# lucidrains/progen

Hardware: NVIDIA H100
Metric: tokens_per_sec (higher is better)
Workload: dtype bf16

## Files before the change

include/progen_b200.h:

```cpp
#ifndef PROGEN_B200_H
#define PROGEN_B200_H
#include <stdint.h>

#ifdef __cplusplus
extern "C" {
#endif

#define PROGEN_F32 0
#define PROGEN_BF16 1

#define PROGEN_BACKEND_SIMT 0
#define PROGEN_BACKEND_TC 1

#define PROGEN_EPI_STORE 0
#define PROGEN_EPI_ROTARY 1
#define PROGEN_EPI_RESIDUAL 2
#define PROGEN_EPI_GLU 3
#define PROGEN_EPI_GELU 4
#define PROGEN_EPI_GLU_BWD 5
#define PROGEN_EPI_GELU_BWD 6
#define PROGEN_EPI_ACCUM 7

const char* progen_version(void);
const char* progen_last_error(void);
// ... 5 lines not shown
  int32_t a_mn_major, b_mn_major;
  int32_t batch;
  int32_t batch_reduce;
  int32_t causal;
  int32_t split_k;
  int32_t in_dtype, out_dtype, epi_kind, backend;
  int32_t seq_len, dim_head;
  int32_t atomic, tril, tril_rows;
  int64_t lda, ldb;
  int64_t a_batch_rows, b_batch_rows, d_batch_rows;
  int64_t ldo, ldo2, ldaux;
  const void* A;
  const void* B;
  void* out;
  void* out2;
  const float* bias;
  const void* aux;
  const float* rot_sin;
  const float* rot_cos;
  float* colsum;
  int64_t lda2, ldb2;
  const void* A2;
  const void* B2;
  int32_t K2, a2_mn_major, b2_mn_major, _pad_tail;
} progen_gemm_t;

int progen_gemm(const progen_gemm_t* desc, void* stream);

int progen_embed_fwd(const int* tokens, const float* table, float* x, long long T, int d, int V, void* stream);
int progen_embed_bwd(const int* tokens, const float* dx, float* dtable, long long T, int d, int V, void* stream);

int progen_ln_shift_fwd(const void* x, long long ldx, int x_dtype, const float* scale, void* y, long long ldy, int y_dtype,
                        float* mean, float* rstd, long long T, int d, int seq_len, int shift, void* stream);
int progen_ln_shift_bwd(const void* dy, long long lddy, int act_dtype, const void* x, long long ldx, int x_dtype,
                        const float* scale, const float* mean, const float* rstd, float* dres, void* dout, long long ldo,
                        float* dscale, float* dres_colsum, long long T, int d, int seq_len, int shift, int residual,
                        void* stream);

int progen_colsum(const void* in, long long ld, int dtype, float* out, long long T, int N, void* stream);

int progen_ce_fwd_bwd(const void* logits, int dtype, const int* labels, float* weights, float* loss, void* dlogits,
                      int dlogits_dtype, int B, int n, int V, float inv_batch, void* stream);

int progen_token_logprob(const void* logits, int dtype, const int* labels, float* logp, float* seq_ll, float* seq_count,
                         int B, int n, int V, void* stream);
int progen_preference_head(const void* logits, int dtype, const int* labels, const float* ref_ll, float* logp, float* seq_ll,
                           float* seq_count, float* weights, float* stats, float* loss, float* ce_scratch, void* dlogits,
// ... 143 lines not shown
```

progen_b200/csrc/api.cu:

```cuda
#include <stdarg.h>
#include "gemm.h"
#include "../../include/progen_b200.h"

static thread_local char g_err[1024] = "";
unsigned long long g_progen_launches = 0;

void progen_set_error(const char* fmt, ...) {
  va_list ap;
  va_start(ap, fmt);
  vsnprintf(g_err, sizeof(g_err), fmt, ap);
  va_end(ap);
}

extern "C" {

const char* progen_version(void) { return "progen_b200 0.1.0 (sm_90a; wgmma/TMA GEMM, CUDA " CUDA_VERSION_STR ")"; }

const char* progen_last_error(void) { return g_err; }

long long progen_launch_count(void) { return (long long)__atomic_load_n(&g_progen_launches, __ATOMIC_RELAXED); }

int progen_device_check(void) {
  int dev = 0;
  PG_CUDA(cudaGetDevice(&dev));
// ... 6 lines not shown
  }
  return PROGEN_OK;
}

int progen_gemm(const progen_gemm_t* d, void* stream) {
  PG_CHECK_ARG(d != nullptr);
  GemmArgs g;
  g.M = d->M; g.N = d->N; g.K = d->K;
  g.A = d->A; g.lda = d->lda; g.a_mn_major = d->a_mn_major;
  g.B = d->B; g.ldb = d->ldb; g.b_mn_major = d->b_mn_major;
  g.batch = d->batch < 1 ? 1 : d->batch;
  g.a_batch_rows = d->a_batch_rows; g.b_batch_rows = d->b_batch_rows; g.d_batch_rows = d->d_batch_rows;
  g.batch_reduce = d->batch_reduce; g.causal = d->causal; g.split_k = d->split_k < 1 ? 1 : d->split_k;
  g.in_dtype = d->in_dtype; g.out_dtype = d->out_dtype; g.epi_kind = d->epi_kind;
  g.epi.out = d->out; g.epi.ldo = d->ldo; g.epi.out2 = d->out2; g.epi.ldo2 = d->ldo2;
  g.epi.bias = d->bias; g.epi.aux = d->aux; g.epi.ldaux = d->ldaux;
  g.epi.rot_sin = d->rot_sin; g.epi.rot_cos = d->rot_cos;
  g.epi.seq_len = d->seq_len > 0 ? d->seq_len : 1; g.epi.dim_head = d->dim_head > 0 ? d->dim_head : 2;
  g.epi.atomic = d->atomic; g.epi.tril = d->tril; g.epi.tril_rows = d->tril_rows > 0 ? d->tril_rows : 1;
  g.epi.colsum = d->colsum;
  g.K2 = d->K2;
  g.A2 = d->A2; g.lda2 = d->lda2; g.a2_mn_major = d->a2_mn_major;
  g.B2 = d->B2; g.ldb2 = d->ldb2; g.b2_mn_major = d->b2_mn_major;
  PG_CHECK_ARG(g.epi_kind >= 0 && g.epi_kind < EPI_NUM_KINDS);
  PG_CHECK_ARG(g.epi.out != nullptr);
  PG_CHECK_ARG(!g.epi.colsum || g.epi_kind == EPI_GLU_BWD || g.epi_kind == EPI_GELU_BWD);
  if (g.epi_kind == EPI_GLU || g.epi_kind == EPI_GELU) PG_CHECK_ARG(g.epi.bias != nullptr);
  if (g.epi_kind == EPI_GLU_BWD || g.epi_kind == EPI_GELU_BWD) PG_CHECK_ARG(g.epi.aux != nullptr);
  if (g.epi_kind == EPI_ROTARY) PG_CHECK_ARG(g.epi.rot_sin && g.epi.rot_cos && d->seq_len > 0 && d->dim_head > 0 && d->dim_head % 2 == 0);
  if (d->backend == PROGEN_BACKEND_TC) return gemm_tc_launch(g, (cudaStream_t)stream);
  if (d->backend == PROGEN_BACKEND_SIMT) return gemm_simt_launch(g, (cudaStream_t)stream);
  progen_set_error("progen_gemm: unknown backend %d", d->backend);
  return PROGEN_ERR_ARG;
}

}
```

progen_b200/csrc/gemm.h:

```cpp
#pragma once
#include "epilogues.cuh"

struct GemmArgs {
  int M, N, K;
  const void* A; long long lda; int a_mn_major;
  const void* B; long long ldb; int b_mn_major;
  int batch; long long a_batch_rows; long long b_batch_rows; long long d_batch_rows;
  int batch_reduce;
  int causal;
  int split_k;
  int in_dtype;
  int out_dtype;
  int epi_kind;
  EpiArgs epi;
  const void* A2; long long lda2; int a2_mn_major;
  const void* B2; long long ldb2; int b2_mn_major;
  int K2;
};

#define PG_CHECK_TAIL(a)                                                                                               \
  do {                                                                                                                 \
    PG_CHECK_ARG((a).K2 >= 0);                                                                                         \
    if ((a).K2 > 0) {                                                                                                  \
      PG_CHECK_ARG((a).A2 != nullptr && (a).B2 != nullptr);                                                            \
      PG_CHECK_ARG((a).split_k == 1 && !(a).causal && (a).batch == 1 && !(a).batch_reduce && (a).epi_kind != EPI_ACCUM); \
    }                                                                                                                  \
  } while (0)

int gemm_tc_launch(const GemmArgs& g, cudaStream_t stream);
int gemm_simt_launch(const GemmArgs& g, cudaStream_t stream);
```

progen_b200/csrc/gemm_tc.cu:

```cuda
#include <cuda.h>
#include <algorithm>
#include <mutex>
#include <unordered_map>
#include "gemm.h"
#include "tc_ptx.cuh"

namespace {

using namespace tc;

constexpr int BM = 128;
constexpr int BN = 128;
constexpr int BK = 64;
constexpr int WG_K = 16;
constexpr int THREADS = 384;
constexpr int A_BYTES = BM * BK * 2;
constexpr int B_BYTES = BN * BK * 2;
constexpr int STAGE_BYTES = A_BYTES + B_BYTES;
constexpr int STAGES = 4;
constexpr int EPI_ROWS = 64;
constexpr int EPI_ITEMS = EPI_ROWS * (BN / 8) / 128;
constexpr int CS_LD = BN + 4;
constexpr int CS_BYTES = EPI_ROWS * CS_LD * 4;
constexpr int SMEM_TOTAL = 1024  + STAGES * STAGE_BYTES + 2 * CS_BYTES + 2 * STAGES * 8;
static_assert(SMEM_TOTAL <= 227 * 1024, "H100: 227 KiB of shared memory per block");
constexpr int BAR_TURN = 1, BAR_EPI = 3;
constexpr int PRODUCER_REGS = 40, CONSUMER_REGS = 232;
static_assert(128 * PRODUCER_REGS + 256 * CONSUMER_REGS <= 65536, "register file");

__device__ __forceinline__ void named_bar_sync(int id, int n) { asm volatile("bar.sync %0, %1;" ::"r"(id), "r"(n) : "memory"); }
__device__ __forceinline__ void named_bar_arrive(int id, int n) { asm volatile("bar.arrive %0, %1;" ::"r"(id), "r"(n) : "memory"); }
template <int R> __device__ __forceinline__ void setmaxnreg_dec() { asm volatile("setmaxnreg.dec.sync.aligned.u32 %0;" ::"n"(R)); }
template <int R> __device__ __forceinline__ void setmaxnreg_inc() { asm volatile("setmaxnreg.inc.sync.aligned.u32 %0;" ::"n"(R)); }

struct GemmDev {
  int M, N, K;
  int batch, batch_reduce;
  int a_batch_rows, b_batch_rows;
  long long d_batch_rows;
  int causal, split_k;
  EpiArgs epi;
  int K2;
};

struct TileInfo {
  int z, m0, n0, kb_begin, kb_end;
  int kb_main;
};

template <bool TAIL>
__device__ __forceinline__ void decode_tile(const GemmDev& g, int t, TileInfo& ti) {
  const int m_tiles = (g.M + BM - 1) / BM;
  const int n_tiles = (g.N + BN - 1) / BN;
  const int per_z = g.split_k * m_tiles * n_tiles;
  ti.z = t / per_z;
  int r = t - ti.z * per_z;
  const int ks = r / (m_tiles * n_tiles);
  r -= ks * (m_tiles * n_tiles);
  ti.m0 = (r / n_tiles) * BM;
  ti.n0 = (r % n_tiles) * BN;
  const int kb_total = (g.K + BK - 1) / BK;
  int b = 0, e = kb_total;
  if (g.causal == 1) e = min(kb_total, (ti.m0 + BM + BK - 1) / BK);
  if (g.causal == 2) b = min(kb_total, ti.m0 / BK);
  if (g.split_k > 1) {
    const int per = (kb_total + g.split_k - 1) / g.split_k;
    b = min(kb_total, ks * per);
    e = min(kb_total, b + per);
  }
  ti.kb_begin = b;
  ti.kb_end = e;
  if constexpr (TAIL) {
    ti.kb_main = e;
    ti.kb_end = e + (g.K2 + BK - 1) / BK;
  }
}

template <bool A_MN, bool B_MN, int KIND, typename TO, bool TAIL>
__global__ void __launch_bounds__(THREADS, 1)
gemm_tc_kernel(const __grid_constant__ CUtensorMap tma_a, const __grid_constant__ CUtensorMap tma_b,
               const __grid_constant__ CUtensorMap tma_a2, const __grid_constant__ CUtensorMap tma_b2, const GemmDev g,
               const int tiles) {
  extern __shared__ uint8_t smem_raw[];
  const uint32_t raw_u32 = smem_u32(smem_raw);
  const uint32_t smem_base = (raw_u32 + 1023u) & ~1023u;
  const uint32_t cs_base = smem_base + STAGES * STAGE_BYTES;
  const uint32_t bar_base = cs_base + 2 * CS_BYTES;
  auto full_bar = [&](int s) { return bar_base + 8u * s; };
  auto empty_bar = [&](int s) { return bar_base + 8u * (STAGES + s); };

  const int wg = threadIdx.x >> 7;
  if (threadIdx.x == 0) {
    prefetch_tensormap(&tma_a);
    prefetch_tensormap(&tma_b);
    if constexpr (TAIL) {
      prefetch_tensormap(&tma_a2);
      prefetch_tensormap(&tma_b2);
    }
    for (int s = 0; s < STAGES; ++s) {
      mbar_init(full_bar(s), 1);
      mbar_init(empty_bar(s), 1);
    }
    fence_barrier_init();
  }
  __syncthreads();

  int stage = 0;
  uint32_t phase = 0;
  auto advance = [&](int n) {
    stage += n;
    phase ^= (uint32_t)(stage / STAGES) & 1u;
    stage %= STAGES;
  };

  if (wg == 0) {
    setmaxnreg_dec<PRODUCER_REGS>();
    if (threadIdx.x == 0) {
      for (int t = blockIdx.x; t < tiles; t += gridDim.x) {
        TileInfo ti;
        decode_tile<TAIL>(g, t, ti);
        const int a_row0 = ti.z * g.a_batch_rows;
        const int b_row0 = ti.z * g.b_batch_rows;
        for (int kb = ti.kb_begin; kb < ti.kb_end; ++kb) {
          mbar_wait(empty_bar(stage), phase ^ 1);
          const uint32_t sa = smem_base + stage * STAGE_BYTES;
          const uint32_t sb = sa + A_BYTES;
          mbar_expect_tx(full_bar(stage), STAGE_BYTES);
          if (TAIL && kb >= ti.kb_main) {
            const int k0 = (kb - ti.kb_main) * BK;
            if constexpr (!A_MN) {
              tma_load_2d(sa, &tma_a2, full_bar(stage), k0, ti.m0);
            } else {
#pragma unroll
              for (int i = 0; i < BM / 64; ++i) tma_load_2d(sa + i * 8192, &tma_a2, full_bar(stage), ti.m0 + 64 * i, k0);
            }
            if constexpr (!B_MN) {
              tma_load_2d(sb, &tma_b2, full_bar(stage), k0, ti.n0);
            } else {
#pragma unroll
              for (int i = 0; i < BN / 64; ++i) tma_load_2d(sb + i * 8192, &tma_b2, full_bar(stage), ti.n0 + 64 * i, k0);
            }
            advance(1);
            continue;
          }
          const int k0 = kb * BK;
          if constexpr (!A_MN) {
            tma_load_2d(sa, &tma_a, full_bar(stage), k0, a_row0 + ti.m0);
          } else {
#pragma unroll
            for (int i = 0; i < BM / 64; ++i)
              tma_load_2d(sa + i * 8192, &tma_a, full_bar(stage), ti.m0 + 64 * i, a_row0 + k0);
          }
          if constexpr (!B_MN) {
            tma_load_2d(sb, &tma_b, full_bar(stage), k0, b_row0 + ti.n0);
          } else {
#pragma unroll
            for (int i = 0; i < BN / 64; ++i)
              tma_load_2d(sb + i * 8192, &tma_b, full_bar(stage), ti.n0 + 64 * i, b_row0 + k0);
          }
          advance(1);
        }
      }
    }
    return;
  }

  setmaxnreg_inc<CONSUMER_REGS>();
  const int c = wg - 1;
  const int tid = threadIdx.x & 127;
  float* cs = reinterpret_cast<float*>(smem_raw + (cs_base - raw_u32)) + c * (CS_BYTES / 4);
  for (int p = 0, t = blockIdx.x; t < tiles; ++p, t += gridDim.x) {
    TileInfo ti;
    decode_tile<TAIL>(g, t, ti);
    if ((p & 1) != c) {
      advance(ti.kb_end - ti.kb_begin);
      continue;
    }
    float acc[2][64];
#pragma unroll
    for (int i = 0; i < 64; ++i) acc[0][i] = acc[1][i] = 0.f;
    if (p > 0) named_bar_sync(BAR_TURN + c, 256);
    int prev = -1;
    for (int kb = ti.kb_begin; kb < ti.kb_end; ++kb) {
      mbar_wait(full_bar(stage), phase);
      const uint32_t sa = smem_base + stage * STAGE_BYTES;
      const uint64_t adesc0 = make_smem_desc<A_MN>(sa), adesc1 = make_smem_desc<A_MN>(sa + 8192);
      const uint64_t bdesc = make_smem_desc<B_MN>(sa + A_BYTES);
      constexpr uint32_t a_step = A_MN ? (2048 >> 4) : (32 >> 4), b_step = B_MN ? (2048 >> 4) : (32 >> 4);
      fence_regs(acc[0]);
      fence_regs(acc[1]);
      wgmma_fence();
#pragma unroll
      for (int k = 0; k < BK / WG_K; ++k) {
        wgmma_m64n128k16_bf16<A_MN ? 1 : 0, B_MN ? 1 : 0>(acc[0], adesc0 + (uint64_t)(k * a_step), bdesc + (uint64_t)(k * b_step));
        wgmma_m64n128k16_bf16<A_MN ? 1 : 0, B_MN ? 1 : 0>(acc[1], adesc1 + (uint64_t)(k * a_step), bdesc + (uint64_t)(k * b_step));
      }
      wgmma_commit();
      fence_regs(acc[0]);
      fence_regs(acc[1]);
      wgmma_wait<1>();
      if (prev >= 0 && tid == 0) mbar_arrive(empty_bar(prev));
      prev = stage;
      advance(1);
    }
    if (t + (int)gridDim.x < tiles) named_bar_arrive(BAR_TURN + (c ^ 1), 256);

    const int w = tid >> 5, lane = tid & 31;
    const int r0 = 16 * w + (lane >> 2), c0 = 2 * (lane & 3);
// ... 121 lines not shown
  cuuint64_t dims[2] = {inner, outer};
  cuuint64_t strides[1] = {row_stride_elems * elem_bytes};
  const CUtensorMapSwizzle sw = swizzle == 128 ? CU_TENSOR_MAP_SWIZZLE_128B : swizzle == 64 ? CU_TENSOR_MAP_SWIZZLE_64B
                              : swizzle == 32 ? CU_TENSOR_MAP_SWIZZLE_32B : CU_TENSOR_MAP_SWIZZLE_NONE;
  cuuint32_t box[2] = {box_inner, box_outer};
  cuuint32_t estr[2] = {1, 1};
  CUtensorMap m;
  CUresult r = fn(&m, elem_bytes == 4 ? CU_TENSOR_MAP_DATA_TYPE_FLOAT32 : CU_TENSOR_MAP_DATA_TYPE_BFLOAT16, 2,
                  const_cast<void*>(ptr), dims, strides, box, estr, CU_TENSOR_MAP_INTERLEAVE_NONE, sw, CU_TENSOR_MAP_L2_PROMOTION_L2_256B,
                  CU_TENSOR_MAP_FLOAT_OOB_FILL_NONE);
  if (r != CUDA_SUCCESS) {
    progen_set_error("cuTensorMapEncodeTiled failed (CUresult %d) ptr=%p inner=%llu outer=%llu stride=%llu box=%ux%u", (int)r,
                     ptr, (unsigned long long)inner, (unsigned long long)outer, (unsigned long long)row_stride_elems,
                     box_inner, box_outer);
    return PROGEN_ERR_CUDA;
  }
  if (cache.size() > 4096) cache.clear();
  cache.emplace(key, m);
  *out = m;
  return PROGEN_OK;
}


template <bool A_MN, bool B_MN, int KIND, typename TO, bool TAIL>
int launch_inst(const CUtensorMap& ta, const CUtensorMap& tb, const CUtensorMap& ta2, const CUtensorMap& tb2,
                const GemmDev& gd, int tiles, cudaStream_t stream) {
  auto kern = gemm_tc_kernel<A_MN, B_MN, KIND, TO, TAIL>;
  static bool attr_set = false;
  if (!attr_set) {
    PG_CUDA(cudaFuncSetAttribute(kern, cudaFuncAttributeMaxDynamicSharedMemorySize, SMEM_TOTAL));
    attr_set = true;
  }
  kern<<<std::min(tiles, pg_num_sms()), THREADS, SMEM_TOTAL, stream>>>(ta, tb, ta2, tb2, gd, tiles);
  PG_LAUNCH_CHECK();
  return PROGEN_OK;
}

}

int pg_tensor_map_2d_bf16(const void* ptr, uint64_t inner, uint64_t outer, uint64_t row_stride_elems, uint32_t box_inner,
                          uint32_t box_outer, CUtensorMap* out) {
  return get_tensor_map(ptr, inner, outer, row_stride_elems, box_inner, box_outer, out);
}

int gemm_tc_launch(const GemmArgs& a, cudaStream_t stream) {
  PG_CHECK_ARG(a.in_dtype == PG_BF16);
  PG_CHECK_ARG(a.M > 0 && a.N > 0 && a.K > 0 && a.batch >= 1 && a.split_k >= 1);
  PG_CHECK_ARG(a.N % 8 == 0);
  PG_CHECK_ARG(a.K % BK == 0);
  PG_CHECK_ARG(a.lda % 8 == 0 && a.ldb % 8 == 0);
  PG_CHECK_ARG((reinterpret_cast<uintptr_t>(a.A) & 15) == 0 && (reinterpret_cast<uintptr_t>(a.B) & 15) == 0);
  PG_CHECK_ARG(!(a.split_k > 1 && a.causal));
  if (a.epi_kind == EPI_ROTARY) PG_CHECK_ARG(a.epi.seq_len % 32 == 0);
  PG_CHECK_ARG((reinterpret_cast<uintptr_t>(a.epi.colsum) & 15) == 0);
  PG_CHECK_ARG(!(a.split_k > 1 || a.batch_reduce) || (a.epi_kind == EPI_ACCUM && a.epi.atomic));
  PG_CHECK_TAIL(a);
  const bool tail = a.K2 > 0;
  if (tail) {
    PG_CHECK_ARG(a.K2 % 8 == 0 && a.lda2 % 8 == 0 && a.ldb2 % 8 == 0);
    PG_CHECK_ARG(a.a2_mn_major == a.a_mn_major && a.b2_mn_major == a.b_mn_major);
    PG_CHECK_ARG((reinterpret_cast<uintptr_t>(a.A2) & 15) == 0 && (reinterpret_cast<uintptr_t>(a.B2) & 15) == 0);
  }

  const uint64_t a_rows = (a.batch > 1 && a.a_batch_rows > 0) ? (uint64_t)a.a_batch_rows * a.batch
                                                              : (uint64_t)(a.a_mn_major ? a.K : a.M);
  const uint64_t b_rows = (a.batch > 1 && a.b_batch_rows > 0) ? (uint64_t)a.b_batch_rows * a.batch
                                                              : (uint64_t)(a.b_mn_major ? a.K : a.N);
  CUtensorMap ta, tb;
  int rc;
  if (!a.a_mn_major) rc = get_tensor_map(a.A, a.K, a_rows, a.lda, BK, BM, &ta);
  else               rc = get_tensor_map(a.A, a.M, a_rows, a.lda, 64, BK, &ta);
  if (rc) return rc;
  if (!a.b_mn_major) rc = get_tensor_map(a.B, a.K, b_rows, a.ldb, BK, BN, &tb);
  else               rc = get_tensor_map(a.B, a.N, b_rows, a.ldb, 64, BK, &tb);
  if (rc) return rc;
  CUtensorMap ta2 = ta, tb2 = tb;
  if (tail) {
    if (!a.a_mn_major) rc = get_tensor_map(a.A2, a.K2, a.M, a.lda2, BK, BM, &ta2);
    else               rc = get_tensor_map(a.A2, a.M, a.K2, a.lda2, 64, BK, &ta2);
    if (rc) return rc;
    if (!a.b_mn_major) rc = get_tensor_map(a.B2, a.K2, a.N, a.ldb2, BK, BN, &tb2);
    else               rc = get_tensor_map(a.B2, a.N, a.K2, a.ldb2, 64, BK, &tb2);
    if (rc) return rc;
  }

  GemmDev gd;
  gd.M = a.M; gd.N = a.N; gd.K = a.K;
  gd.batch = a.batch; gd.batch_reduce = a.batch_reduce;
  gd.a_batch_rows = (int)a.a_batch_rows; gd.b_batch_rows = (int)a.b_batch_rows; gd.d_batch_rows = a.d_batch_rows;
  gd.causal = a.causal; gd.split_k = a.split_k;
  gd.epi = a.epi;
  gd.K2 = a.K2;
  const long long tiles = (long long)a.batch * a.split_k * ((a.M + BM - 1) / BM) * ((a.N + BN - 1) / BN);
  PG_CHECK_ARG(tiles < (1ll << 31));

  const int am = a.a_mn_major ? 1 : 0, bm = a.b_mn_major ? 1 : 0;
  const bool obf = a.out_dtype == PG_BF16;
#define TC_CASE(AM, BMJ, KIND, TO)                                                                       \
  return tail ? launch_inst<AM, BMJ, KIND, TO, true>(ta, tb, ta2, tb2, gd, (int)tiles, stream)            \
              : launch_inst<AM, BMJ, KIND, TO, false>(ta, tb, ta2, tb2, gd, (int)tiles, stream)
  switch (a.epi_kind) {
    case EPI_STORE:
      if (!am && bm) { if (obf) TC_CASE(false, true, EPI_STORE, bf16); else TC_CASE(false, true, EPI_STORE, float); }
      if (!am && !bm) { if (obf) TC_CASE(false, false, EPI_STORE, bf16); else TC_CASE(false, false, EPI_STORE, float); }
      if (am && bm) { if (obf) TC_CASE(true, true, EPI_STORE, bf16); else TC_CASE(true, true, EPI_STORE, float); }
      break;
    case EPI_ROTARY:
      if (!am && bm && obf) TC_CASE(false, true, EPI_ROTARY, bf16);
      break;
    case EPI_RESIDUAL:
      if (!am && bm) TC_CASE(false, true, EPI_RESIDUAL, float);
      break;
    case EPI_GLU:
      if (!am && bm && obf) TC_CASE(false, true, EPI_GLU, bf16);
      break;
    case EPI_GELU:
      if (!am && bm && obf) TC_CASE(false, true, EPI_GELU, bf16);
      break;
    case EPI_GLU_BWD:
      if (!am && !bm && obf) TC_CASE(false, false, EPI_GLU_BWD, bf16);
      break;
    case EPI_GELU_BWD:
      if (!am && !bm && obf) TC_CASE(false, false, EPI_GELU_BWD, bf16);
      break;
    case EPI_ACCUM:
      if (am && bm) return launch_inst<true, true, EPI_ACCUM, float, false>(ta, tb, ta2, tb2, gd, (int)tiles, stream);
      if (!am && !bm) return launch_inst<false, false, EPI_ACCUM, float, false>(ta, tb, ta2, tb2, gd, (int)tiles, stream);
      break;
    default: break;
  }
#undef TC_CASE
  progen_set_error("gemm_tc: unsupported combination epi=%d a_mn=%d b_mn=%d out=%d", a.epi_kind, am, bm, a.out_dtype);
  return PROGEN_ERR_UNSUPPORTED;
}
```

progen_b200/csrc/tc_ptx.cuh:

```cuda
#pragma once
#include <cuda.h>
#include "common.cuh"

namespace tc {

__device__ __forceinline__ uint32_t smem_u32(const void* p) { return (uint32_t)__cvta_generic_to_shared(p); }

__device__ __forceinline__ void mbar_init(uint32_t bar, uint32_t count) {
  asm volatile("mbarrier.init.shared::cta.b64 [%0], %1;" ::"r"(bar), "r"(count) : "memory");
}
__device__ __forceinline__ void mbar_expect_tx(uint32_t bar, uint32_t bytes) {
  asm volatile("mbarrier.arrive.expect_tx.shared::cta.b64 _, [%0], %1;" ::"r"(bar), "r"(bytes) : "memory");
}
__device__ __forceinline__ void mbar_arrive(uint32_t bar) {
  asm volatile("mbarrier.arrive.shared::cta.b64 _, [%0];" ::"r"(bar) : "memory");
}
__device__ __forceinline__ void mbar_wait(uint32_t bar, uint32_t parity) {
  uint32_t ok = 0, spins = 0;
  do {
    asm volatile(
        "{\n\t.reg .pred p;\n\t"
        "mbarrier.try_wait.parity.shared::cta.b64 p, [%1], %2;\n\t"
        "selp.u32 %0, 1, 0, p;\n\t}"
        : "=r"(ok) : "r"(bar), "r"(parity) : "memory");
// ... 30 lines not shown
  for (int i = 0; i < R; ++i) asm volatile("" : "+f"(d[i])::"memory");
}

template <int TA, int TB>
__device__ __forceinline__ void wgmma_m64n128k16_bf16(float (&d)[64], uint64_t adesc, uint64_t bdesc) {
  asm volatile(
      "{\n\t"
      "wgmma.mma_async.sync.aligned.m64n128k16.f32.bf16.bf16 "
      "{%0, %1, %2, %3, %4, %5, %6, %7, %8, %9, %10, %11, %12, %13, %14, %15, %16, %17, %18, %19, %20, %21, %22, %23, "
      "%24, %25, %26, %27, %28, %29, %30, %31, %32, %33, %34, %35, %36, %37, %38, %39, %40, %41, %42, %43, %44, %45, %46, "
      "%47, %48, %49, %50, %51, %52, %53, %54, %55, %56, %57, %58, %59, %60, %61, %62, %63}, "
      "%64, %65, 1, 1, 1, %66, %67;\n\t}"
      : "+f"(d[0]), "+f"(d[1]), "+f"(d[2]), "+f"(d[3]), "+f"(d[4]), "+f"(d[5]), "+f"(d[6]), "+f"(d[7]), "+f"(d[8]),
        "+f"(d[9]), "+f"(d[10]), "+f"(d[11]), "+f"(d[12]), "+f"(d[13]), "+f"(d[14]), "+f"(d[15]), "+f"(d[16]),
        "+f"(d[17]), "+f"(d[18]), "+f"(d[19]), "+f"(d[20]), "+f"(d[21]), "+f"(d[22]), "+f"(d[23]), "+f"(d[24]),
        "+f"(d[25]), "+f"(d[26]), "+f"(d[27]), "+f"(d[28]), "+f"(d[29]), "+f"(d[30]), "+f"(d[31]), "+f"(d[32]),
        "+f"(d[33]), "+f"(d[34]), "+f"(d[35]), "+f"(d[36]), "+f"(d[37]), "+f"(d[38]), "+f"(d[39]), "+f"(d[40]),
        "+f"(d[41]), "+f"(d[42]), "+f"(d[43]), "+f"(d[44]), "+f"(d[45]), "+f"(d[46]), "+f"(d[47]), "+f"(d[48]),
        "+f"(d[49]), "+f"(d[50]), "+f"(d[51]), "+f"(d[52]), "+f"(d[53]), "+f"(d[54]), "+f"(d[55]), "+f"(d[56]),
        "+f"(d[57]), "+f"(d[58]), "+f"(d[59]), "+f"(d[60]), "+f"(d[61]), "+f"(d[62]), "+f"(d[63])
      : "l"(adesc), "l"(bdesc), "n"(TA), "n"(TB));
}

template <int TB>
__device__ __forceinline__ void wgmma_m64n64k16_ss(float (&d)[32], uint64_t adesc, uint64_t bdesc) {
  asm volatile(
      "{\n\t"
      "wgmma.mma_async.sync.aligned.m64n64k16.f32.bf16.bf16 "
      "{%0, %1, %2, %3, %4, %5, %6, %7, %8, %9, %10, %11, %12, %13, %14, %15, %16, %17, %18, %19, %20, %21, %22, %23, %24, %25, %26, %27, %28, %29, %30, %31}, "
      "%32, %33, 1, 1, 1, 0, %34;\n\t}"
      : "+f"(d[0]), "+f"(d[1]), "+f"(d[2]), "+f"(d[3]), "+f"(d[4]), "+f"(d[5]), "+f"(d[6]), "+f"(d[7]), "+f"(d[8]), "+f"(d[9]), "+f"(d[10]), "+f"(d[11]), "+f"(d[12]), "+f"(d[13]), "+f"(d[14]), "+f"(d[15]), "+f"(d[16]), "+f"(d[17]), "+f"(d[18]), "+f"(d[19]), "+f"(d[20]), "+f"(d[21]), "+f"(d[22]), "+f"(d[23]), "+f"(d[24]), "+f"(d[25]), "+f"(d[26]), "+f"(d[27]), "+f"(d[28]), "+f"(d[29]), "+f"(d[30]), "+f"(d[31])
      : "l"(adesc), "l"(bdesc), "n"(TB));
}
template <int TB>
__device__ __forceinline__ void wgmma_m64n64k16_rs(float (&d)[32], const uint32_t (&a)[4], uint64_t bdesc) {
  asm volatile(
      "{\n\t"
      "wgmma.mma_async.sync.aligned.m64n64k16.f32.bf16.bf16 "
      "{%0, %1, %2, %3, %4, %5, %6, %7, %8, %9, %10, %11, %12, %13, %14, %15, %16, %17, %18, %19, %20, %21, %22, %23, %24, %25, %26, %27, %28, %29, %30, %31}, "
      "{%32, %33, %34, %35}, %36, 1, 1, 1, %37;\n\t}"
      : "+f"(d[0]), "+f"(d[1]), "+f"(d[2]), "+f"(d[3]), "+f"(d[4]), "+f"(d[5]), "+f"(d[6]), "+f"(d[7]), "+f"(d[8]), "+f"(d[9]), "+f"(d[10]), "+f"(d[11]), "+f"(d[12]), "+f"(d[13]), "+f"(d[14]), "+f"(d[15]), "+f"(d[16]), "+f"(d[17]), "+f"(d[18]), "+f"(d[19]), "+f"(d[20]), "+f"(d[21]), "+f"(d[22]), "+f"(d[23]), "+f"(d[24]), "+f"(d[25]), "+f"(d[26]), "+f"(d[27]), "+f"(d[28]), "+f"(d[29]), "+f"(d[30]), "+f"(d[31])
      : "r"(a[0]), "r"(a[1]), "r"(a[2]), "r"(a[3]), "l"(bdesc), "n"(TB));
}

}

// ... 3 lines not shown
```

progen_b200/engine.py:

```python
import math
import numpy as np
import torch

from . import lib as L

P = 'pro_gen_base/~/'
ALIGN = 64


CUT_ALIGN = 128


def counted_length(labels):
    labels = np.asarray(labels)
    n = labels.shape[1]
    pad = labels == 0
    first = np.where(pad.any(1), pad.argmax(1), n)
    last = np.where((~pad).any(1), n - 1 - (~pad)[:, ::-1].argmax(1), -1)
    return np.minimum(n, np.maximum(first, last) + 1)


def cut_length(labels):
    n = np.asarray(labels).shape[1]
    need = int(counted_length(labels).max()) if len(labels) else 1
    return min(n, -(-need // CUT_ALIGN) * CUT_ALIGN)


def check_length(labels, length, what):
    labels = np.asarray(labels)
    n = labels.shape[1]
    if length is None:
        return cut_length(labels)
    if isinstance(length, (bool, np.bool_)) or not isinstance(length, (int, np.integer)) or \
# ... 317 lines not shown
        if lo is None:
            return {}
        seg = lo.layout.seg
        g, A = lo.g[:acts.T], seg(lo.lp, module, 'lora_a')
        self.dgrad_gemm(dy, N, seg(lo.lp, module, 'lora_b'), lo.r, g, acts=acts)
        self.wgrad_gemm(lo.u[module][:acts.T], lo.r, dy, N, seg(lo.grads, module, 'lora_b'), acts=acts)
        self.wgrad_gemm(x, K, g, lo.r, seg(lo.grads, module, 'lora_a'), acts=acts)
        return dict(A2=g, lda2=lo.r, B2=A, ldb2=lo.r, K2=lo.r)

    def fwd_gemm(self, x, K, w, N, out, epi=L.EPI_STORE, out_dtype=None, acts=None, **kw):
        self._mm(M=(acts or self.acts).T, N=N, K=K, A=x, lda=K, B=w, ldb=N, b_mn=True, out=out, ldo=kw.pop('ldo', N), epi=epi,
                 out_dtype=self.act_dt if out_dtype is None else out_dtype, **kw)

    def dgrad_gemm(self, dy, N_out, w, K_in, out, epi=L.EPI_STORE, acts=None, **kw):
        self._mm(M=(acts or self.acts).T, N=K_in, K=N_out, A=dy, lda=N_out, B=w, ldb=N_out, out=out, ldo=kw.pop('ldo', K_in), epi=epi,
                 out_dtype=self.act_dt, **kw)

    def wgrad_gemm(self, x, K_in, dy, N_out, dw, acts=None):
        split = self.wgrad_split(K_in, N_out, acts) if self.backend == L.BACKEND_TC else 1
        self._mm(M=K_in, N=N_out, K=(acts or self.acts).T, A=x, lda=K_in, a_mn=True, B=dy, ldb=N_out, b_mn=True, out=dw, ldo=N_out,
                 epi=L.EPI_ACCUM, out_dtype=L.F32, split_k=split, atomic=split > 1)

    def wgrad_split(self, K_in, N_out, acts=None):
        tiles = ((K_in + 127) // 128) * ((N_out + 127) // 128)
        fill = lambda s: tiles * s / (-(-tiles * s // self.num_sms) * self.num_sms)
        return max(range(1, min(8, max(1, (acts or self.acts).T // 64)) + 1), key=lambda s: (round(fill(s), 6), -s))

    def colsum(self, t, N, out, ld=None, acts=None):
        L.check(self.lib.progen_colsum(t.data_ptr(), N if ld is None else ld, L.dt(t), out.data_ptr(), (acts or self.acts).T, N,
                                       L.stream()), 'colsum')

    def ln_fwd(self, x, ldx, scale, y, ldy, mean, rstd, dcols, shift, acts=None):
        a = acts or self.acts
        L.check(self.lib.progen_ln_shift_fwd(x.data_ptr(), ldx, L.dt(x), scale.data_ptr(), y.data_ptr(), ldy, L.dt(y),
                                             mean.data_ptr(), rstd.data_ptr(), a.T, dcols, a.n, int(shift), L.stream()),
                'ln_fwd')

    def forward(self, ids):
        B = ids.shape[0]
        self.ensure_batch(B)
        self.tok.copy_(torch.as_tensor(ids).reshape(-1).to(device=self.dev, dtype=torch.int32), non_blocking=True)
        self._forward_device()
        return self.logits

    def prefill(self, ids, P, sink):
        Bs = ids.shape[0]
        if tuple(ids.shape[1:]) != (self.n,) or not 0 < P < self.n:
            raise L.ProgenError(f'prefill: ids must be (B, {self.n}) and 0 < P < {self.n}')
        acts = self.inference_acts(Bs)
# ... 426 lines not shown
```

progen_b200/lib.py:

```python
import ctypes as C
import os
import torch

F32, BF16 = 0, 1
BACKEND_SIMT, BACKEND_TC = 0, 1
EPI_STORE, EPI_ROTARY, EPI_RESIDUAL, EPI_GLU, EPI_GELU, EPI_GLU_BWD, EPI_GELU_BWD, EPI_ACCUM = range(8)
TASK_REGRESSION, TASK_CLASSIFICATION = 0, 1
PROPERTY_MAX_OUTPUTS = 64

_HERE = os.path.dirname(os.path.abspath(__file__))
LIB_PATH = os.path.join(_HERE, 'libprogen_b200.so')


class ProgenError(RuntimeError):
    pass


class GemmDesc(C.Structure):
    _fields_ = [
        ('M', C.c_int32), ('N', C.c_int32), ('K', C.c_int32),
        ('a_mn_major', C.c_int32), ('b_mn_major', C.c_int32),
        ('batch', C.c_int32), ('batch_reduce', C.c_int32), ('causal', C.c_int32), ('split_k', C.c_int32),
        ('in_dtype', C.c_int32), ('out_dtype', C.c_int32), ('epi_kind', C.c_int32), ('backend', C.c_int32),
        ('seq_len', C.c_int32), ('dim_head', C.c_int32),
        ('atomic', C.c_int32), ('tril', C.c_int32), ('tril_rows', C.c_int32),
        ('lda', C.c_int64), ('ldb', C.c_int64),
        ('a_batch_rows', C.c_int64), ('b_batch_rows', C.c_int64), ('d_batch_rows', C.c_int64),
        ('ldo', C.c_int64), ('ldo2', C.c_int64), ('ldaux', C.c_int64),
        ('A', C.c_void_p), ('B', C.c_void_p), ('out', C.c_void_p), ('out2', C.c_void_p),
        ('bias', C.c_void_p), ('aux', C.c_void_p), ('rot_sin', C.c_void_p), ('rot_cos', C.c_void_p),
        ('colsum', C.c_void_p),
        ('lda2', C.c_int64), ('ldb2', C.c_int64), ('A2', C.c_void_p), ('B2', C.c_void_p),
        ('K2', C.c_int32), ('a2_mn_major', C.c_int32), ('b2_mn_major', C.c_int32), ('_pad_tail', C.c_int32),
    ]


_lib = None

_LL, _I, _P, _F = C.c_longlong, C.c_int, C.c_void_p, C.c_float

PROTOTYPES = {
    'progen_version': [],
    'progen_last_error': [],
    'progen_device_check': [],
    'progen_launch_count': [],
    'progen_gemm': [C.POINTER(GemmDesc), _P],
    'progen_embed_fwd': [_P, _P, _P, _LL, _I, _I, _P],
    'progen_embed_bwd': [_P, _P, _P, _LL, _I, _I, _P],
    'progen_ln_shift_fwd': [_P, _LL, _I, _P, _P, _LL, _I, _P, _P, _LL, _I, _I, _I, _P],
    'progen_ln_shift_bwd': [_P, _LL, _I, _P, _LL, _I, _P, _P, _P, _P, _P, _LL, _P, _P, _LL, _I, _I, _I, _I, _P],
    'progen_colsum': [_P, _LL, _I, _P, _LL, _I, _P],
    'progen_ce_fwd_bwd': [_P, _I, _P, _P, _P, _P, _I, _I, _I, _I, _F, _P],
    'progen_token_logprob': [_P, _I, _P, _P, _P, _P, _I, _I, _I, _P],
    'progen_preference_head': [_P, _I, _P, _P, _P, _P, _P, _P, _P, _P, _P, _P, _I, _I, _I, _I, _F, _F, _P],
    'progen_masked_mean_pool': [_P, _LL, _I, _P, _P, _I, _I, _I, _P],
    'progen_masked_mean_pool_bwd': [_P, _P, _P, _LL, _I, _I, _I, _I, _P],
# ... 52 lines not shown
        raise ProgenError('no CUDA device: progen_b200 has no CPU fallback (sm_90a only)')
    check(load().progen_device_check(), 'progen_device_check')


def dt(t):
    if t.dtype == torch.float32:
        return F32
    if t.dtype == torch.bfloat16:
        return BF16
    raise ProgenError(f'unsupported dtype {t.dtype}')


def ptr(t):
    return 0 if t is None else t.data_ptr()


def stream():
    return torch.cuda.current_stream().cuda_stream


def gemm(*, M, N, K, A, lda, B, ldb, out, ldo, epi=EPI_STORE, backend, a_mn=False, b_mn=False, in_dtype, out_dtype=F32,
         batch=1, a_batch_rows=0, b_batch_rows=0, d_batch_rows=0, batch_reduce=False, causal=0, split_k=1,
         out2=None, ldo2=0, bias=None, aux=None, ldaux=0, rot_sin=None, rot_cos=None, seq_len=0, dim_head=0,
         atomic=False, tril=False, tril_rows=0, colsum=None, A2=None, lda2=0, a2_mn=None, B2=None, ldb2=0, b2_mn=None, K2=0):
    d = GemmDesc()
    d.M, d.N, d.K = M, N, K
    d.a_mn_major, d.b_mn_major = int(a_mn), int(b_mn)
    d.batch, d.batch_reduce, d.causal, d.split_k = batch, int(batch_reduce), causal, split_k
    d.in_dtype, d.out_dtype, d.epi_kind, d.backend = in_dtype, out_dtype, epi, backend
    d.seq_len, d.dim_head = seq_len, dim_head
    d.atomic, d.tril, d.tril_rows = int(atomic), int(tril), tril_rows
    d.lda, d.ldb = lda, ldb
    d.a_batch_rows, d.b_batch_rows, d.d_batch_rows = a_batch_rows, b_batch_rows, d_batch_rows
    d.ldo, d.ldo2, d.ldaux = ldo, ldo2, ldaux
    as_ptr = lambda x: x if isinstance(x, int) else ptr(x)
    d.A, d.B, d.out, d.out2 = as_ptr(A), as_ptr(B), as_ptr(out), as_ptr(out2)
    d.bias, d.aux, d.rot_sin, d.rot_cos = as_ptr(bias), as_ptr(aux), as_ptr(rot_sin), as_ptr(rot_cos)
    d.colsum = as_ptr(colsum)
    if K2:
        d.K2, d.lda2, d.ldb2, d.A2, d.B2 = K2, lda2, ldb2, as_ptr(A2), as_ptr(B2)
        d.a2_mn_major = int(a_mn if a2_mn is None else a2_mn)
        d.b2_mn_major = int(b_mn if b2_mn is None else b2_mn)
    check(load().progen_gemm(C.byref(d), stream()), 'progen_gemm')
```

Measured before the change: 1.021 million.

## Add 128x256 wide-tile wgmma path for weight-gradient accumulate GEMMs

Adds a wide-N (256) tile variant of the TMA/wgmma GEMM for MN-major EPI_ACCUM weight-gradient GEMMs. Both consumer warpgroups cooperate on one 128x256 tile using m64n256k16 instructions and write straight from registers to global memory (atomic or read-modify-write), with no shared-memory staging. This should raise operand reuse per byte loaded and reduce the number of tiles. The split-K heuristic is also replaced with a cost model that charges each wave a fixed overhead and allows splits up to 16. The trade-offs are 128-register accumulators, uncoalesced direct stores, and more split-K atomics.

```diff
diff --git a/include/progen_b200.h b/include/progen_b200.h
--- a/include/progen_b200.h
+++ b/include/progen_b200.h
@@ -51,7 +51,8 @@
   int64_t lda2, ldb2;
   const void* A2;
   const void* B2;
-  int32_t K2, a2_mn_major, b2_mn_major, _pad_tail;
+  int32_t K2, a2_mn_major, b2_mn_major;
+  int32_t tile_n;
 } progen_gemm_t;
 
 int progen_gemm(const progen_gemm_t* desc, void* stream);
diff --git a/progen_b200/csrc/api.cu b/progen_b200/csrc/api.cu
--- a/progen_b200/csrc/api.cu
+++ b/progen_b200/csrc/api.cu
@@ -52,6 +52,7 @@
   g.K2 = d->K2;
   g.A2 = d->A2; g.lda2 = d->lda2; g.a2_mn_major = d->a2_mn_major;
   g.B2 = d->B2; g.ldb2 = d->ldb2; g.b2_mn_major = d->b2_mn_major;
+  g.tile_n = d->tile_n;
   PG_CHECK_ARG(g.epi_kind >= 0 && g.epi_kind < EPI_NUM_KINDS);
   PG_CHECK_ARG(g.epi.out != nullptr);
   PG_CHECK_ARG(!g.epi.colsum || g.epi_kind == EPI_GLU_BWD || g.epi_kind == EPI_GELU_BWD);
diff --git a/progen_b200/csrc/gemm.h b/progen_b200/csrc/gemm.h
--- a/progen_b200/csrc/gemm.h
+++ b/progen_b200/csrc/gemm.h
@@ -16,6 +16,7 @@
   const void* A2; long long lda2; int a2_mn_major;
   const void* B2; long long ldb2; int b2_mn_major;
   int K2;
+  int tile_n;
 };
 
 #define PG_CHECK_TAIL(a)                                                                                               \
diff --git a/progen_b200/csrc/gemm_tc.cu b/progen_b200/csrc/gemm_tc.cu
--- a/progen_b200/csrc/gemm_tc.cu
+++ b/progen_b200/csrc/gemm_tc.cu
@@ -11,6 +11,7 @@
 
 constexpr int BM = 128;
 constexpr int BN = 128;
+constexpr int BN_WIDE = 2 * BN;
 constexpr int BK = 64;
 constexpr int WG_K = 16;
 constexpr int THREADS = 384;
@@ -24,6 +25,11 @@
 constexpr int CS_BYTES = EPI_ROWS * CS_LD * 4;
 constexpr int SMEM_TOTAL = 1024  + STAGES * STAGE_BYTES + 2 * CS_BYTES + 2 * STAGES * 8;
 static_assert(SMEM_TOTAL <= 227 * 1024, "H100: 227 KiB of shared memory per block");
+constexpr int STAGE_BYTES_WIDE = A_BYTES + BN_WIDE * BK * 2;
+constexpr int SMEM_WIDE = 1024 + STAGES * STAGE_BYTES_WIDE + 2 * STAGES * 8;
+static_assert(SMEM_WIDE <= 227 * 1024, "H100: 227 KiB of shared memory per block");
+template <int TN> constexpr int stage_bytes() { return TN == BN ? STAGE_BYTES : STAGE_BYTES_WIDE; }
+template <int TN> constexpr int smem_bytes() { return TN == BN ? SMEM_TOTAL : SMEM_WIDE; }
 constexpr int BAR_TURN = 1, BAR_EPI = 3;
 constexpr int PRODUCER_REGS = 40, CONSUMER_REGS = 232;
 static_assert(128 * PRODUCER_REGS + 256 * CONSUMER_REGS <= 65536, "register file");
@@ -48,17 +54,17 @@
   int kb_main;
 };
 
-template <bool TAIL>
+template <bool TAIL, int TN>
 __device__ __forceinline__ void decode_tile(const GemmDev& g, int t, TileInfo& ti) {
   const int m_tiles = (g.M + BM - 1) / BM;
-  const int n_tiles = (g.N + BN - 1) / BN;
+  const int n_tiles = (g.N + TN - 1) / TN;
   const int per_z = g.split_k * m_tiles * n_tiles;
   ti.z = t / per_z;
   int r = t - ti.z * per_z;
   const int ks = r / (m_tiles * n_tiles);
   r -= ks * (m_tiles * n_tiles);
   ti.m0 = (r / n_tiles) * BM;
-  ti.n0 = (r % n_tiles) * BN;
+  ti.n0 = (r % n_tiles) * TN;
   const int kb_total = (g.K + BK - 1) / BK;
   int b = 0, e = kb_total;
   if (g.causal == 1) e = min(kb_total, (ti.m0 + BM + BK - 1) / BK);
@@ -76,16 +82,19 @@
   }
 }
 
-template <bool A_MN, bool B_MN, int KIND, typename TO, bool TAIL>
+template <bool A_MN, bool B_MN, int KIND, typename TO, bool TAIL, int TN>
 __global__ void __launch_bounds__(THREADS, 1)
 gemm_tc_kernel(const __grid_constant__ CUtensorMap tma_a, const __grid_constant__ CUtensorMap tma_b,
                const __grid_constant__ CUtensorMap tma_a2, const __grid_constant__ CUtensorMap tma_b2, const GemmDev g,
                const int tiles) {
+  constexpr bool WIDE = TN == BN_WIDE;
+  static_assert(TN == BN || (WIDE && A_MN && B_MN && KIND == EPI_ACCUM && !TAIL), "the wide tile is the weight gradient's");
+  constexpr int STAGE_B = stage_bytes<TN>();
   extern __shared__ uint8_t smem_raw[];
   const uint32_t raw_u32 = smem_u32(smem_raw);
   const uint32_t smem_base = (raw_u32 + 1023u) & ~1023u;
-  const uint32_t cs_base = smem_base + STAGES * STAGE_BYTES;
-  const uint32_t bar_base = cs_base + 2 * CS_BYTES;
+  const uint32_t cs_base = smem_base + STAGES * STAGE_B;
+  const uint32_t bar_base = cs_base + (WIDE ? 0 : 2 * CS_BYTES);
   auto full_bar = [&](int s) { return bar_base + 8u * s; };
   auto empty_bar = [&](int s) { return bar_base + 8u * (STAGES + s); };
 
@@ -99,7 +108,7 @@
     }
     for (int s = 0; s < STAGES; ++s) {
       mbar_init(full_bar(s), 1);
-      mbar_init(empty_bar(s), 1);
+      mbar_init(empty_bar(s), WIDE ? 2 : 1);
     }
     fence_barrier_init();
   }
@@ -118,14 +127,14 @@
     if (threadIdx.x == 0) {
       for (int t = blockIdx.x; t < tiles; t += gridDim.x) {
         TileInfo ti;
-        decode_tile<TAIL>(g, t, ti);
+        decode_tile<TAIL, TN>(g, t, ti);
         const int a_row0 = ti.z * g.a_batch_rows;
         const int b_row0 = ti.z * g.b_batch_rows;
         for (int kb = ti.kb_begin; kb < ti.kb_end; ++kb) {
           mbar_wait(empty_bar(stage), phase ^ 1);
-          const uint32_t sa = smem_base + stage * STAGE_BYTES;
+          const uint32_t sa = smem_base + stage * STAGE_B;
           const uint32_t sb = sa + A_BYTES;
-          mbar_expect_tx(full_bar(stage), STAGE_BYTES);
+          mbar_expect_tx(full_bar(stage), STAGE_B);
           if (TAIL && kb >= ti.kb_main) {
             const int k0 = (kb - ti.kb_main) * BK;
             if constexpr (!A_MN) {
@@ -155,7 +164,7 @@
             tma_load_2d(sb, &tma_b, full_bar(stage), k0, b_row0 + ti.n0);
           } else {
 #pragma unroll
-            for (int i = 0; i < BN / 64; ++i)
+            for (int i = 0; i < TN / 64; ++i)
               tma_load_2d(sb + i * 8192, &tma_b, full_bar(stage), ti.n0 + 64 * i, b_row0 + k0);
           }
           advance(1);
@@ -168,10 +177,61 @@
   setmaxnreg_inc<CONSUMER_REGS>();
   const int c = wg - 1;
   const int tid = threadIdx.x & 127;
+  if constexpr (WIDE) {
+    const int w = tid >> 5, lane = tid & 31;
+    for (int t = blockIdx.x; t < tiles; t += gridDim.x) {
+      TileInfo ti;
+      decode_tile<false, TN>(g, t, ti);
+      float acc[128];
+#pragma unroll
+      for (int i = 0; i < 128; ++i) acc[i] = 0.f;
+      int prev = -1;
+      for (int kb = ti.kb_begin; kb < ti.kb_end; ++kb) {
+        mbar_wait(full_bar(stage), phase);
+        const uint32_t sa = smem_base + stage * STAGE_B;
+        const uint64_t adesc = make_smem_desc<true>(sa + c * 8192), bdesc = make_smem_desc<true>(sa + A_BYTES);
+        fence_regs(acc);
+        wgmma_fence();
+#pragma unroll
+        for (int k = 0; k < BK / WG_K; ++k)
+          wgmma_m64n256k16_bf16<1, 1>(acc, adesc + (uint64_t)(k * (2048 >> 4)), bdesc + (uint64_t)(k * (2048 >> 4)));
+        wgmma_commit();
+        fence_regs(acc);
+        wgmma_wait<1>();
+        if (prev >= 0 && tid == 0) mbar_arrive(empty_bar(prev));
+        prev = stage;
+        advance(1);
+      }
+      wgmma_wait<0>();
+      fence_regs(acc);
+      if (prev >= 0 && tid == 0) mbar_arrive(empty_bar(prev));
+      const int row = ti.m0 + 64 * c + 16 * w + (lane >> 2), col = ti.n0 + 2 * (lane & 3);
+#pragma unroll
+      for (int h = 0; h < 2; ++h) {
+        if (row + 8 * h >= g.M) continue;
+        float* po = reinterpret_cast<float*>(g.epi.out) + (long long)(row + 8 * h) * g.epi.ldo + col;
+#pragma unroll
+        for (int j = 0; j < 32; ++j) {
+          if (col + 8 * j >= g.N) continue;
+          const float x = acc[4 * j + 2 * h], y = acc[4 * j + 2 * h + 1];
+          if (g.epi.atomic) {
+            asm volatile("red.global.add.v2.f32 [%0], {%1, %2};" ::"l"(po + 8 * j), "f"(x), "f"(y) : "memory");
+          } else {
+            float2 o = *reinterpret_cast<const float2*>(po + 8 * j);
+            o.x += x;
+            o.y += y;
+            *reinterpret_cast<float2*>(po + 8 * j) = o;
+          }
+        }
+      }
+    }
+    return;
+  }
+
   float* cs = reinterpret_cast<float*>(smem_raw + (cs_base - raw_u32)) + c * (CS_BYTES / 4);
   for (int p = 0, t = blockIdx.x; t < tiles; ++p, t += gridDim.x) {
     TileInfo ti;
-    decode_tile<TAIL>(g, t, ti);
+    decode_tile<TAIL, TN>(g, t, ti);
     if ((p & 1) != c) {
       advance(ti.kb_end - ti.kb_begin);
       continue;
@@ -183,7 +243,7 @@
     int prev = -1;
     for (int kb = ti.kb_begin; kb < ti.kb_end; ++kb) {
       mbar_wait(full_bar(stage), phase);
-      const uint32_t sa = smem_base + stage * STAGE_BYTES;
+      const uint32_t sa = smem_base + stage * STAGE_B;
       const uint64_t adesc0 = make_smem_desc<A_MN>(sa), adesc1 = make_smem_desc<A_MN>(sa + 8192);
       const uint64_t bdesc = make_smem_desc<B_MN>(sa + A_BYTES);
       constexpr uint32_t a_step = A_MN ? (2048 >> 4) : (32 >> 4), b_step = B_MN ? (2048 >> 4) : (32 >> 4);
@@ -351,16 +411,16 @@
 }
 
 
-template <bool A_MN, bool B_MN, int KIND, typename TO, bool TAIL>
+template <bool A_MN, bool B_MN, int KIND, typename TO, bool TAIL, int TN = BN>
 int launch_inst(const CUtensorMap& ta, const CUtensorMap& tb, const CUtensorMap& ta2, const CUtensorMap& tb2,
                 const GemmDev& gd, int tiles, cudaStream_t stream) {
-  auto kern = gemm_tc_kernel<A_MN, B_MN, KIND, TO, TAIL>;
+  auto kern = gemm_tc_kernel<A_MN, B_MN, KIND, TO, TAIL, TN>;
   static bool attr_set = false;
   if (!attr_set) {
-    PG_CUDA(cudaFuncSetAttribute(kern, cudaFuncAttributeMaxDynamicSharedMemorySize, SMEM_TOTAL));
+    PG_CUDA(cudaFuncSetAttribute(kern, cudaFuncAttributeMaxDynamicSharedMemorySize, smem_bytes<TN>()));
     attr_set = true;
   }
-  kern<<<std::min(tiles, pg_num_sms()), THREADS, SMEM_TOTAL, stream>>>(ta, tb, ta2, tb2, gd, tiles);
+  kern<<<std::min(tiles, pg_num_sms()), THREADS, smem_bytes<TN>(), stream>>>(ta, tb, ta2, tb2, gd, tiles);
   PG_LAUNCH_CHECK();
   return PROGEN_OK;
 }
@@ -384,6 +444,7 @@
   PG_CHECK_ARG((reinterpret_cast<uintptr_t>(a.epi.colsum) & 15) == 0);
   PG_CHECK_ARG(!(a.split_k > 1 || a.batch_reduce) || (a.epi_kind == EPI_ACCUM && a.epi.atomic));
   PG_CHECK_TAIL(a);
+  PG_CHECK_ARG(a.tile_n == 0 || a.tile_n == BN);
   const bool tail = a.K2 > 0;
   if (tail) {
     PG_CHECK_ARG(a.K2 % 8 == 0 && a.lda2 % 8 == 0 && a.ldb2 % 8 == 0);
@@ -420,7 +481,10 @@
   gd.causal = a.causal; gd.split_k = a.split_k;
   gd.epi = a.epi;
   gd.K2 = a.K2;
-  const long long tiles = (long long)a.batch * a.split_k * ((a.M + BM - 1) / BM) * ((a.N + BN - 1) / BN);
+  const bool wide = a.tile_n == 0 && a.epi_kind == EPI_ACCUM && a.a_mn_major && a.b_mn_major && !tail && a.batch == 1 &&
+                    !a.epi.tril && a.N >= BN_WIDE;
+  const int tn = wide ? BN_WIDE : BN;
+  const long long tiles = (long long)a.batch * a.split_k * ((a.M + BM - 1) / BM) * ((a.N + tn - 1) / tn);
   PG_CHECK_ARG(tiles < (1ll << 31));
 
   const int am = a.a_mn_major ? 1 : 0, bm = a.b_mn_major ? 1 : 0;
@@ -453,7 +517,10 @@
       if (!am && !bm && obf) TC_CASE(false, false, EPI_GELU_BWD, bf16);
       break;
     case EPI_ACCUM:
-      if (am && bm) return launch_inst<true, true, EPI_ACCUM, float, false>(ta, tb, ta2, tb2, gd, (int)tiles, stream);
+      if (am && bm) {
+        if (wide) return launch_inst<true, true, EPI_ACCUM, float, false, BN_WIDE>(ta, tb, ta2, tb2, gd, (int)tiles, stream);
+        return launch_inst<true, true, EPI_ACCUM, float, false>(ta, tb, ta2, tb2, gd, (int)tiles, stream);
+      }
       if (!am && !bm) return launch_inst<false, false, EPI_ACCUM, float, false>(ta, tb, ta2, tb2, gd, (int)tiles, stream);
       break;
     default: break;
diff --git a/progen_b200/csrc/tc_ptx.cuh b/progen_b200/csrc/tc_ptx.cuh
--- a/progen_b200/csrc/tc_ptx.cuh
+++ b/progen_b200/csrc/tc_ptx.cuh
@@ -76,6 +76,38 @@
       : "l"(adesc), "l"(bdesc), "n"(TA), "n"(TB));
 }
 
+template <int TA, int TB>
+__device__ __forceinline__ void wgmma_m64n256k16_bf16(float (&d)[128], uint64_t adesc, uint64_t bdesc) {
+  asm volatile(
+      "{\n\t"
+      "wgmma.mma_async.sync.aligned.m64n256k16.f32.bf16.bf16 "
+      "{%0, %1, %2, %3, %4, %5, %6, %7, %8, %9, %10, %11, %12, %13, %14, %15, %16, %17, %18, %19, %20, %21, %22, %23, "
+      "%24, %25, %26, %27, %28, %29, %30, %31, %32, %33, %34, %35, %36, %37, %38, %39, %40, %41, %42, %43, %44, %45, "
+      "%46, %47, %48, %49, %50, %51, %52, %53, %54, %55, %56, %57, %58, %59, %60, %61, %62, %63, %64, %65, %66, %67, "
+      "%68, %69, %70, %71, %72, %73, %74, %75, %76, %77, %78, %79, %80, %81, %82, %83, %84, %85, %86, %87, %88, %89, "
+      "%90, %91, %92, %93, %94, %95, %96, %97, %98, %99, %100, %101, %102, %103, %104, %105, %106, %107, %108, %109, "
+      "%110, %111, %112, %113, %114, %115, %116, %117, %118, %119, %120, %121, %122, %123, %124, %125, %126, %127}, "
+      "%128, %129, 1, 1, 1, %130, %131;\n\t}"
+      : "+f"(d[0]), "+f"(d[1]), "+f"(d[2]), "+f"(d[3]), "+f"(d[4]), "+f"(d[5]), "+f"(d[6]), "+f"(d[7]), "+f"(d[8]),
+        "+f"(d[9]), "+f"(d[10]), "+f"(d[11]), "+f"(d[12]), "+f"(d[13]), "+f"(d[14]), "+f"(d[15]), "+f"(d[16]),
+        "+f"(d[17]), "+f"(d[18]), "+f"(d[19]), "+f"(d[20]), "+f"(d[21]), "+f"(d[22]), "+f"(d[23]), "+f"(d[24]),
+        "+f"(d[25]), "+f"(d[26]), "+f"(d[27]), "+f"(d[28]), "+f"(d[29]), "+f"(d[30]), "+f"(d[31]), "+f"(d[32]),
+        "+f"(d[33]), "+f"(d[34]), "+f"(d[35]), "+f"(d[36]), "+f"(d[37]), "+f"(d[38]), "+f"(d[39]), "+f"(d[40]),
+        "+f"(d[41]), "+f"(d[42]), "+f"(d[43]), "+f"(d[44]), "+f"(d[45]), "+f"(d[46]), "+f"(d[47]), "+f"(d[48]),
+        "+f"(d[49]), "+f"(d[50]), "+f"(d[51]), "+f"(d[52]), "+f"(d[53]), "+f"(d[54]), "+f"(d[55]), "+f"(d[56]),
+        "+f"(d[57]), "+f"(d[58]), "+f"(d[59]), "+f"(d[60]), "+f"(d[61]), "+f"(d[62]), "+f"(d[63]), "+f"(d[64]),
+        "+f"(d[65]), "+f"(d[66]), "+f"(d[67]), "+f"(d[68]), "+f"(d[69]), "+f"(d[70]), "+f"(d[71]), "+f"(d[72]),
+        "+f"(d[73]), "+f"(d[74]), "+f"(d[75]), "+f"(d[76]), "+f"(d[77]), "+f"(d[78]), "+f"(d[79]), "+f"(d[80]),
+        "+f"(d[81]), "+f"(d[82]), "+f"(d[83]), "+f"(d[84]), "+f"(d[85]), "+f"(d[86]), "+f"(d[87]), "+f"(d[88]),
+        "+f"(d[89]), "+f"(d[90]), "+f"(d[91]), "+f"(d[92]), "+f"(d[93]), "+f"(d[94]), "+f"(d[95]), "+f"(d[96]),
+        "+f"(d[97]), "+f"(d[98]), "+f"(d[99]), "+f"(d[100]), "+f"(d[101]), "+f"(d[102]), "+f"(d[103]), "+f"(d[104]),
+        "+f"(d[105]), "+f"(d[106]), "+f"(d[107]), "+f"(d[108]), "+f"(d[109]), "+f"(d[110]), "+f"(d[111]),
+        "+f"(d[112]), "+f"(d[113]), "+f"(d[114]), "+f"(d[115]), "+f"(d[116]), "+f"(d[117]), "+f"(d[118]),
+        "+f"(d[119]), "+f"(d[120]), "+f"(d[121]), "+f"(d[122]), "+f"(d[123]), "+f"(d[124]), "+f"(d[125]),
+        "+f"(d[126]), "+f"(d[127])
+      : "l"(adesc), "l"(bdesc), "n"(TA), "n"(TB));
+}
+
 template <int TB>
 __device__ __forceinline__ void wgmma_m64n64k16_ss(float (&d)[32], uint64_t adesc, uint64_t bdesc) {
   asm volatile(
diff --git a/progen_b200/engine.py b/progen_b200/engine.py
--- a/progen_b200/engine.py
+++ b/progen_b200/engine.py
@@ -9,6 +9,7 @@
 
 
 CUT_ALIGN = 128
+WGRAD_UNIT_KBLOCKS = 32
 
 
 def counted_length(labels):
@@ -372,9 +373,11 @@
                  epi=L.EPI_ACCUM, out_dtype=L.F32, split_k=split, atomic=split > 1)
 
     def wgrad_split(self, K_in, N_out, acts=None):
-        tiles = ((K_in + 127) // 128) * ((N_out + 127) // 128)
-        fill = lambda s: tiles * s / (-(-tiles * s // self.num_sms) * self.num_sms)
-        return max(range(1, min(8, max(1, (acts or self.acts).T // 64)) + 1), key=lambda s: (round(fill(s), 6), -s))
+        tn = 256 if N_out >= 256 else 128
+        tiles = ((K_in + 127) // 128) * ((N_out + tn - 1) // tn)
+        kb = -(-(acts or self.acts).T // 64)
+        cost = lambda s: -(-tiles * s // self.num_sms) * (-(-kb // s) + WGRAD_UNIT_KBLOCKS)
+        return min(range(1, min(16, kb) + 1), key=lambda s: (cost(s), s))
 
     def colsum(self, t, N, out, ld=None, acts=None):
         L.check(self.lib.progen_colsum(t.data_ptr(), N if ld is None else ld, L.dt(t), out.data_ptr(), (acts or self.acts).T, N,
diff --git a/progen_b200/lib.py b/progen_b200/lib.py
--- a/progen_b200/lib.py
+++ b/progen_b200/lib.py
@@ -31,7 +31,7 @@
         ('bias', C.c_void_p), ('aux', C.c_void_p), ('rot_sin', C.c_void_p), ('rot_cos', C.c_void_p),
         ('colsum', C.c_void_p),
         ('lda2', C.c_int64), ('ldb2', C.c_int64), ('A2', C.c_void_p), ('B2', C.c_void_p),
-        ('K2', C.c_int32), ('a2_mn_major', C.c_int32), ('b2_mn_major', C.c_int32), ('_pad_tail', C.c_int32),
+        ('K2', C.c_int32), ('a2_mn_major', C.c_int32), ('b2_mn_major', C.c_int32), ('tile_n', C.c_int32),
     ]
 
 
@@ -130,7 +130,8 @@
 def gemm(*, M, N, K, A, lda, B, ldb, out, ldo, epi=EPI_STORE, backend, a_mn=False, b_mn=False, in_dtype, out_dtype=F32,
          batch=1, a_batch_rows=0, b_batch_rows=0, d_batch_rows=0, batch_reduce=False, causal=0, split_k=1,
          out2=None, ldo2=0, bias=None, aux=None, ldaux=0, rot_sin=None, rot_cos=None, seq_len=0, dim_head=0,
-         atomic=False, tril=False, tril_rows=0, colsum=None, A2=None, lda2=0, a2_mn=None, B2=None, ldb2=0, b2_mn=None, K2=0):
+         atomic=False, tril=False, tril_rows=0, colsum=None, A2=None, lda2=0, a2_mn=None, B2=None, ldb2=0, b2_mn=None, K2=0,
+         tile_n=0):
     d = GemmDesc()
     d.M, d.N, d.K = M, N, K
     d.a_mn_major, d.b_mn_major = int(a_mn), int(b_mn)
@@ -145,6 +146,7 @@
     d.A, d.B, d.out, d.out2 = as_ptr(A), as_ptr(B), as_ptr(out), as_ptr(out2)
     d.bias, d.aux, d.rot_sin, d.rot_cos = as_ptr(bias), as_ptr(aux), as_ptr(rot_sin), as_ptr(rot_cos)
     d.colsum = as_ptr(colsum)
+    d.tile_n = tile_n
     if K2:
         d.K2, d.lda2, d.ldb2, d.A2, d.B2 = K2, lda2, ldb2, as_ptr(A2), as_ptr(B2)
         d.a2_mn_major = int(a_mn if a2_mn is None else a2_mn)
```

Result: faster. 1.040 million, median of 6 (+1.9%).
